# 0xC000005/PyChebyshev

Hardware: AMD Instinct MI355X
Metric: point-evals/sec, 5D Black-Scholes n=11^5 barycentric + TT, 1/2/4/8 GPU (higher is better)
Workload: dtype f64; 1 GPU; 5D Black-Scholes n=11^5 full-tensor barycentric, 1,000,000 fp64 queries per GPU; evals_per_point=1, parallelism=batch-sharded x1, model replicated, one process per GPU, gather=none

## Files before the change

### pychebyshev_amd/csrc/bary_kernels.h

```cpp
#pragma once

#include <type_traits>

#include "pcx_common.h"

static __global__ void k_mode_product(const double *__restrict__ in, double *__restrict__ out,
                               const double *__restrict__ D, long outer, int na, long inner) {
    long idx = (long)blockIdx.x * blockDim.x + threadIdx.x;
    long total = outer * na * inner;
    if (idx >= total) return;
    long q = idx % inner;
    long t = idx / inner;
    int i = (int)(t % na);
    long o = t / na;
    const double *src = in + (o * na) * inner + q;
    const double *drow = D + (long)i * na;
    double s = 0.0;
    for (int j = 0; j < na; ++j) s = __builtin_fma(src[(long)j * inner], drow[j], s);
    out[idx] = s;
}

static __global__ void k_contract_axis(const double *__restrict__ in, double *__restrict__ out,
                                const double *__restrict__ vec, long outer, int na, long inner) {
    long idx = (long)blockIdx.x * blockDim.x + threadIdx.x;
    if (idx >= outer * inner) return;
    long q = idx % inner;
    long o = idx / inner;
    const double *src = in + (o * na) * inner + q;
    double s = 0.0;
    for (int j = 0; j < na; ++j) s = __builtin_fma(src[(long)j * inner], vec[j], s);
    out[idx] = s;
}

static __global__ void k_pack_fragments(const double *__restrict__ T2, double *__restrict__ frag, int M,
                                 int K, int MT, int KS, int R) {
    long idx = (long)blockIdx.x * blockDim.x + threadIdx.x;
    long total = (long)MT * KS * 64;
    if (idx >= total) return;
    int l = (int)(idx & 63);
    long ts = idx >> 6;
    int s = (int)(ts % KS);
    int t = (int)(ts / KS);
    int m = 16 * t + (l & 15);
    int k = R + 4 * s + (l >> 4);
    frag[idx] = (m < M && k < K) ? T2[(long)m * K + k] : 0.0;
}

static __global__ void k_pack_seed(const double *__restrict__ T2, double *__restrict__ seed, int M, int K, int MT, int R, int tps) {
    long idx = (long)blockIdx.x * blockDim.x + threadIdx.x;
    if (idx >= (long)MT * 16 * R) return;
    const int j = (int)(idx & 3);
    const int r = (int)((idx >> 2) % R);
    const long tg = (idx >> 2) / R;
    const int g = (int)(tg & 3);
    const long t = tg >> 2;
    const long slab = tps > 0 ? t / tps : 0;
    const int m = 16 * (int)(tps > 0 ? t % tps : t) + g + 4 * j;
    seed[idx] = m < M ? T2[(slab * M + m) * K + r] : 0.0;
}

static __global__ void k_pack_fragments_slabs(const double *__restrict__ T3, double *__restrict__ frag, int n0, int M1,
                                       int K, int tps, int KS, int R) {
    long idx = (long)blockIdx.x * blockDim.x + threadIdx.x;
    const long per_slab = (long)tps * KS * 64;
    if (idx >= per_slab * n0) return;
    const int i0 = (int)(idx / per_slab);
    const long r = idx - (long)i0 * per_slab;
    int l = (int)(r & 63);
    long ts = r >> 6;
    int s = (int)(ts % KS);
    int t = (int)(ts / KS);
    int m = 16 * t + (l & 15);
    int k = R + 4 * s + (l >> 4);
    frag[idx] = (m < M1 && k < K) ? T3[((long)i0 * M1 + m) * K + k] : 0.0;
}

__device__ __forceinline__ void bary_g0_finish(const BaryG0 &gs, const double *__restrict__ diff0, double *vecA,
                                               double *vecB, const double *b0, int stride, double *out_row) {
    typedef const double __attribute__((address_space(4))) *cptr_t;
    const cptr_t D0 = (cptr_t)(unsigned long long)diff0;
    const int n0 = gs.n0;
    for (int o = 0; o <= gs.maxorder; ++o) {
        if (o > 0) {
            for (int i = 0; i < n0; ++i) {
                double s = 0.0;
                for (int j = 0; j < n0; ++j) s = __builtin_fma(vecA[j * stride], D0[i * n0 + j], s);
                vecB[i * stride] = s;
            }
            double *t = vecA; vecA = vecB; vecB = t;
        }
        double y = 0.0;
        for (int i = 0; i < n0; ++i) y = __builtin_fma(b0[i * stride], vecA[i * stride], y);
        if (out_row)
            for (int s = 0; s < gs.nmem; ++s)
                if (gs.order[s] == o) out_row[gs.col[s]] = y;
    }
}

__device__ __forceinline__ void bary_weights_1d(double x, const double *__restrict__ nodes,
                                                const double *__restrict__ wts, int n, double *dst,
                                                int stride) {
    int exact = -1;
    for (int j = 0; j < n; ++j) {
        double diff = x - nodes[j];
        if (exact < 0 && __builtin_fabs(diff) < 1e-14) exact = j;
    }
    if (exact >= 0) {
        for (int j = 0; j < n; ++j) dst[j * stride] = (j == exact) ? 1.0 : 0.0;
    } else {
        double su = 0.0;
        for (int j = 0; j < n; ++j) {
            double u = wts[j] / (x - nodes[j]);
            dst[j * stride] = u;
            su += u;
        }
        double r = 1.0 / su;
        for (int j = 0; j < n; ++j) dst[j * stride] *= r;
    }
}

__device__ __forceinline__ double code_weight(unsigned code, const double *bw_col, int PW) {
    double w0 = bw_col[(code & 255u) * PW];
    double w1 = bw_col[((code >> 8) & 255u) * PW];
    double w2 = bw_col[((code >> 16) & 255u) * PW];
    double w3 = bw_col[(code >> 24) * PW];
    return (w0 * w1) * (w2 * w3);
}

struct pcx_u4 { unsigned v[4]; };
__device__ __forceinline__ pcx_u4 load_row_codes(const unsigned *__restrict__ codes, long t, int g) {
    const uint4 q = reinterpret_cast<const uint4 *>(codes)[4 * t + g];
    return pcx_u4{{q.x, q.y, q.z, q.w}};
}

typedef const pcx_d4 __attribute__((address_space(1))) *pcx_seed_ptr;
template <int R>
struct pcx_seed { pcx_d4 v[R > 0 ? R : 1]; };
template <int R>
__device__ __forceinline__ pcx_seed<R> load_seed(pcx_seed_ptr seed, long t, int g) {
    pcx_seed<R> q;
#pragma unroll
    for (int r = 0; r < R; ++r) q.v[r] = seed[(4 * t + g) * R + r];
    return q;
}

__device__ __forceinline__ pcx_u4 load_row_offs(const unsigned *__restrict__ offs, long t, int g, int w) {
    const uint4 q = reinterpret_cast<const uint4 *>(offs)[8 * t + 2 * g + w];
    return pcx_u4{{q.x, q.y, q.z, q.w}};
}

template <int NF>
__device__ __forceinline__ double code_weight_t(unsigned code, const double *bw_col, int PW) {
    if constexpr (NF >= 4) return code_weight(code, bw_col, PW);
    else {
        double w0 = bw_col[(code & 255u) * PW];
        double w1 = bw_col[((code >> 8) & 255u) * PW];
        if constexpr (NF == 3) return (w0 * w1) * bw_col[((code >> 16) & 255u) * PW];
        else return w0 * w1;
    }
}

#define PCX_CHUNK_TILES 4

template <int KS, int NT, bool WIDE, int NF = 4, bool G0 = false, int R = 0>
__global__ void __launch_bounds__(256, 2)
k_bary_mfma(BaryDims dims, BaryMfmaPlan plan, const double *__restrict__ nodes,
            const double *__restrict__ wts, const double *const *__restrict__ frag_tab,
            const unsigned *__restrict__ rowcode, const unsigned *__restrict__ kcode,
            const unsigned *__restrict__ rowcode_hi, const unsigned *__restrict__ kcode_hi,
            const double *__restrict__ pts, double *__restrict__ out, long N, long ostride,
            long ooff, int chunks_per_split, double *__restrict__ partial,
            const int *__restrict__ perm, BaryG0 gs, const double *__restrict__ diff0,
            const unsigned *__restrict__ rowoff, BaryTail tail) {
    static_assert(NT == 1 || NT == 2 || NT == 4, "PW must divide the wave");
    constexpr int PW = 16 * NT;
    constexpr int PH = 64 / PW;
    extern __shared__ double lds[];
    const int lane = threadIdx.x & 63;
    const int wave = threadIdx.x >> 6;
    const int g = lane >> 4;
    const int c = lane & 15;
    double *bw = lds + (size_t)wave * plan.rows * PW;
    const double *bwt = bw + (size_t)plan.tail_base * PW;
    int bx = blockIdx.x;
    const int nchunks = (plan.MT + PCX_CHUNK_TILES - 1) / PCX_CHUNK_TILES;
    int ch0 = blockIdx.y * chunks_per_split, ch_len = chunks_per_split;
    bool split = gridDim.y > 1;
    long part_p0 = 0;
    long part_n = N;
    if (!G0 && tail.P > 0 && bx >= tail.first) {
        const int e = bx - tail.first;
        const int tb = e / tail.P;
        bx = tail.first + tb;
        ch0 = (e - tb * tail.P) * tail.cpp;
        ch_len = tail.cpp;
        split = true;
        part_p0 = (long)tail.first * 4 * PW;
        part_n = N - part_p0;
    }
    const int ch1 = (ch0 + ch_len < nchunks) ? ch0 + ch_len : nchunks;
    const long base = ((long)bx * 4 + wave) * PW;
    typedef const double __attribute__((address_space(1))) *gptr_t;
    const gptr_t frag = (gptr_t)frag_tab[blockIdx.z];
    const pcx_seed_ptr seed = (pcx_seed_ptr)(frag + (size_t)plan.MT * KS * 64);

    {
        const int pp = lane % PW;
        const int ph = lane / PW;
        const long pidx = base + pp;
        const bool valid = pidx < N;
        const long row = valid ? (perm ? (long)perm[pidx] : pidx) : 0;
        for (int k = ph; k < dims.d; k += PH) {
            const double *nd = nodes + dims.off[k];
            double x = valid ? pts[row * dims.d + k] : nd[0];
            const int trow = dims.off[k] + (k >= plan.split ? 1 : 0);
            bary_weights_1d(x, nd, wts + dims.off[k], dims.n[k], bw + (size_t)trow * PW + pp, PW);
        }
        if (ph == 0) {
            bw[(size_t)(plan.tail_base - 1) * PW + pp] = 1.0;
            bw[(size_t)(plan.rows - 1) * PW + pp] = 1.0;
        }
    }
    __syncthreads();

    double B[NT][KS];
    double ws[NT][R > 0 ? R : 1];
    auto tail_weights = [&](auto nft) {
        constexpr int NFT = decltype(nft)::value;
#pragma unroll
        for (int s = 0; s < KS; ++s) {
            unsigned code = kcode[4 * s + g];
#pragma unroll
            for (int nt = 0; nt < NT; ++nt) B[nt][s] = code_weight_t<NFT>(code, bwt + 16 * nt + c, PW);
            if (WIDE) {
                unsigned hi = kcode_hi[4 * s + g];
#pragma unroll
                for (int nt = 0; nt < NT; ++nt) B[nt][s] *= code_weight(hi, bwt + 16 * nt + c, PW);
            }
        }
#pragma unroll
        for (int r = 0; r < R; ++r) {
            unsigned code = kcode[4 * KS + r];
#pragma unroll
            for (int nt = 0; nt < NT; ++nt) ws[nt][r] = code_weight_t<NFT>(code, bwt + 16 * nt + c, PW);
            if (WIDE) {
                unsigned hi = kcode_hi[4 * KS + r];
#pragma unroll
                for (int nt = 0; nt < NT; ++nt) ws[nt][r] *= code_weight(hi, bwt + 16 * nt + c, PW);
            }
        }
    };
    if (!WIDE && dims.d - plan.split <= 2) tail_weights(std::integral_constant<int, 2>{});
    else tail_weights(std::integral_constant<int, 4>{});

    double total[NT], cs[NT];
#pragma unroll
    for (int nt = 0; nt < NT; ++nt) { total[nt] = 0.0; cs[nt] = 0.0; }
    const gptr_t tf = frag + lane;
    const int t_begin = ch0 * PCX_CHUNK_TILES;
    const int t_end = (ch1 * PCX_CHUNK_TILES < plan.MT) ? ch1 * PCX_CHUNK_TILES : plan.MT;
    constexpr bool PIPELINED = (KS >= 12);
    constexpr int DEPTH = 6;
    constexpr bool OFFS = PIPELINED && !WIDE && !G0;
    constexpr bool CODE2 = WIDE || (OFFS && NF >= 3);
    constexpr int CODE_STEP = 8;
    unsigned cc[4] = {0u, 0u, 0u, 0u}, cch[4] = {0u, 0u, 0u, 0u};
    auto load_codes = [&](long t) {
        const pcx_u4 q = OFFS ? load_row_offs(rowoff, t, g, 0) : load_row_codes(rowcode, t, g);
        pcx_u4 qh = q;
        if constexpr (WIDE) qh = load_row_codes(rowcode_hi, t, g);
        else if constexpr (CODE2) qh = load_row_offs(rowoff, t, g, 1);
#pragma unroll
        for (int j = 0; j < 4; ++j) {
            cc[j] = q.v[j];
            if (CODE2) cch[j] = qh.v[j];
        }
    };
    auto head_entry = [&](int j, int nt, int f) -> double {
        if constexpr (OFFS) {
            const unsigned word = f < 2 ? cc[j] : cch[j];
            const unsigned off = (f & 1) ? (word >> 16) : (word & 0xffffu);
            return *reinterpret_cast<const double *>(reinterpret_cast<const char *>(bw + 16 * nt + c) + off);
        } else {
            return bw[(size_t)((cc[j] >> (8 * f)) & 255u) * PW + 16 * nt + c];
        }
    };
    double head[DEPTH];
    pcx_d4 acc[NT];
    auto seed_acc = [&](const pcx_seed<R> &sd) {
#pragma unroll
        for (int nt = 0; nt < NT; ++nt) acc[nt] = (pcx_d4){0.0, 0.0, 0.0, 0.0};
#pragma unroll
        for (int r = 0; r < R; ++r)
#pragma unroll
            for (int nt = 0; nt < NT; ++nt)
#pragma unroll
                for (int j = 0; j < 4; ++j) acc[nt][j] = __builtin_fma(sd.v[r][j], ws[nt][r], acc[nt][j]);
    };
    constexpr bool CARRY = PIPELINED && R > 0;
#pragma unroll
    for (int i = 0; i < DEPTH; ++i) head[i] = 0.0;
    if (PIPELINED && t_begin < t_end) {
        if constexpr (R > 0) seed_acc(load_seed<R>(seed, t_begin, g));
        load_codes(t_begin);
#pragma unroll
        for (int i = 0; i < DEPTH; ++i) head[i] = tf[((size_t)t_begin * KS + i) * 64];
    }
    for (int t = t_begin; t < t_end; ++t) {
        double w[NT][4];
        pcx_seed<R> sdn;
        if constexpr (!CARRY) {
            if constexpr (R > 0) sdn = load_seed<R>(seed, t, g);
            seed_acc(sdn);
        }
        const gptr_t tt = tf + (size_t)t * KS * 64;
        if constexpr (PIPELINED) {
            const int t_next = (t + 1 < t_end) ? t + 1 : t;
            const gptr_t tn = tf + (size_t)t_next * KS * 64;
            double ring[DEPTH];
#pragma unroll
            for (int i = 0; i < DEPTH; ++i) ring[i] = head[i];
            double wr[4][NT][4];
            double wh[4][NT][4];
#pragma unroll
            for (int s = 0; s < KS; ++s) {
                const double a = ring[s % DEPTH];
                if (s + DEPTH < KS) ring[s % DEPTH] = tt[(s + DEPTH) * 64];
                else head[s + DEPTH - KS] = tn[(s + DEPTH - KS) * 64];
                if constexpr (R > 0) {
                    if (s == KS - DEPTH) sdn = load_seed<R>(seed, t_next, g);
                }
                if (s == CODE_STEP) load_codes(t_next);
#pragma unroll
                for (int j = 0; j < 4; ++j) {
                    if (s == 2 * j) {
#pragma unroll
                        for (int nt = 0; nt < NT; ++nt)
#pragma unroll
                            for (int f = 0; f < (NF < 4 ? NF : 4); ++f)
                                wr[j][nt][f] = head_entry(j, nt, f);
                    }
                    if (s == 2 * j + 2) {
#pragma unroll
                        for (int nt = 0; nt < NT; ++nt)
                            w[nt][j] = NF >= 4 ? (wr[j][nt][0] * wr[j][nt][1]) * (wr[j][nt][2] * wr[j][nt][3])
                                     : (NF == 3 ? (wr[j][nt][0] * wr[j][nt][1]) * wr[j][nt][2]
                                                : wr[j][nt][0] * wr[j][nt][1]);
                    }
                    if (WIDE && s == 2 * j + 1) {
#pragma unroll
                        for (int nt = 0; nt < NT; ++nt)
#pragma unroll
                            for (int f = 0; f < 4; ++f)
                                wh[j][nt][f] = bw[(size_t)((cch[j] >> (8 * f)) & 255u) * PW + 16 * nt + c];
                    }
                    if (WIDE && s == 2 * j + 3) {
#pragma unroll
                        for (int nt = 0; nt < NT; ++nt)
                            w[nt][j] *= (wh[j][nt][0] * wh[j][nt][1]) * (wh[j][nt][2] * wh[j][nt][3]);
                    }
                }
                __builtin_amdgcn_sched_barrier(0);
#pragma unroll
                for (int nt = 0; nt < NT; ++nt)
                    acc[nt] = __builtin_amdgcn_mfma_f64_16x16x4f64(a, B[nt][s], acc[nt], 0, 0, 0);
                __builtin_amdgcn_sched_barrier(0);
            }
        } else {
            const pcx_u4 q = load_row_codes(rowcode, t, g);
            pcx_u4 qh = q;
            if (WIDE) qh = load_row_codes(rowcode_hi, t, g);
#pragma unroll
            for (int j = 0; j < 4; ++j) {
                unsigned code = q.v[j];
#pragma unroll
                for (int nt = 0; nt < NT; ++nt) w[nt][j] = code_weight_t<NF>(code, bw + 16 * nt + c, PW);
                if (WIDE) {
                    unsigned hi = qh.v[j];
#pragma unroll
                    for (int nt = 0; nt < NT; ++nt) w[nt][j] *= code_weight(hi, bw + 16 * nt + c, PW);
                }
            }
#pragma unroll
            for (int s = 0; s < KS; ++s) {
                double a = tt[s * 64];
#pragma unroll
                for (int nt = 0; nt < NT; ++nt)
                    acc[nt] = __builtin_amdgcn_mfma_f64_16x16x4f64(a, B[nt][s], acc[nt], 0, 0, 0);
            }
        }
#pragma unroll
        for (int nt = 0; nt < NT; ++nt)
#pragma unroll
            for (int j = 0; j < 4; ++j) cs[nt] = __builtin_fma(acc[nt][j], w[nt][j], cs[nt]);
        if constexpr (CARRY) seed_acc(sdn);
        if constexpr (G0) {
            if ((t + 1) % gs.tps == 0) {
                const int i0 = t / gs.tps;
                double *Pl = const_cast<double *>(bwt);
#pragma unroll
                for (int nt = 0; nt < NT; ++nt) {
                    double v = cs[nt];
                    v += __shfl_xor(v, 16, 64);
                    v += __shfl_xor(v, 32, 64);
                    if (g == 0) Pl[(size_t)i0 * PW + 16 * nt + c] = v;
                    cs[nt] = 0.0;
                }
            }
            continue;
        }
        const bool chunk_end = ((t + 1) % PCX_CHUNK_TILES == 0) || (t + 1 == plan.MT);
        if (chunk_end) {
            if (split) {
                const int ch = t / PCX_CHUNK_TILES;
#pragma unroll
                for (int nt = 0; nt < NT; ++nt) {
                    long pidx = base + 16 * nt + c;
                    if (pidx < N)
                        partial[(((size_t)blockIdx.z * nchunks + ch) * 4 + g) * (size_t)part_n + (pidx - part_p0)] = cs[nt];
                }
            }
#pragma unroll
            for (int nt = 0; nt < NT; ++nt) { total[nt] += cs[nt]; cs[nt] = 0.0; }
        }
    }

    if constexpr (G0) {
        if (lane < PW) {
            double *Pl = const_cast<double *>(bwt) + lane;
            const long pidx = base + lane;
            const long row = (pidx < N) ? (perm ? (long)perm[pidx] : pidx) : 0;
            bary_g0_finish(gs, diff0, Pl, Pl + (size_t)gs.n0 * PW, bw + (size_t)dims.off[0] * PW + lane, PW,
                           pidx < N ? out + row * ostride + ooff : nullptr);
        }
        return;
    }
    if (!split) {
#pragma unroll
        for (int nt = 0; nt < NT; ++nt) {
            double v = total[nt];
            v += __shfl_xor(v, 16, 64);
            v += __shfl_xor(v, 32, 64);
            long pidx = base + 16 * nt + c;
            if (g == 0 && pidx < N) {
                long row = perm ? (long)perm[pidx] : pidx;
                out[row * ostride + ooff + blockIdx.z] = v;
            }
        }
    }
}

template <int KS, int R = 0>
__global__ void __launch_bounds__(512, 2)
k_bary_mfma4(BaryDims dims, BaryMfmaPlan plan, const double *__restrict__ nodes,
             const double *__restrict__ wts, const double *const *__restrict__ frag_tab,
             const unsigned *__restrict__ rowcode, const unsigned *__restrict__ kcode,
             const double *__restrict__ pts, double *__restrict__ out, long N, long ostride,
             long ooff, const int *__restrict__ perm) {
    constexpr int NT = 2;
    constexpr int PW = 32;
    constexpr int SLAB = KS * 64;
    constexpr int CPT = (SLAB + 511) / 512;
    extern __shared__ double lds[];
    const int lane = threadIdx.x & 63;
    const int wave = threadIdx.x >> 6;
    const int g = lane >> 4;
    const int c = lane & 15;
    double *bw = lds + (size_t)wave * plan.rows * PW;
    const double *bwt = bw + (size_t)plan.tail_base * PW;
    double *slab = lds + (size_t)8 * plan.rows * PW;
    const long base = ((long)blockIdx.x * 8 + wave) * PW;
    typedef const double __attribute__((address_space(1))) *gptr_t;
    const gptr_t frag = (gptr_t)frag_tab[blockIdx.z];
    const pcx_seed_ptr seed = (pcx_seed_ptr)(frag + (size_t)plan.MT * SLAB);

    {
        const int pp = lane & 31;
        const int ph = lane >> 5;
        const long pidx = base + pp;
        const bool valid = pidx < N;
        const long row = valid ? (perm ? (long)perm[pidx] : pidx) : 0;
        for (int k = ph; k < dims.d; k += 2) {
            const double *nd = nodes + dims.off[k];
            double x = valid ? pts[row * dims.d + k] : nd[0];
            const int trow = dims.off[k] + (k >= plan.split ? 1 : 0);
            bary_weights_1d(x, nd, wts + dims.off[k], dims.n[k], bw + (size_t)trow * PW + pp, PW);
        }
        if (ph == 0) {
            bw[(size_t)(plan.tail_base - 1) * PW + pp] = 1.0;
            bw[(size_t)(plan.rows - 1) * PW + pp] = 1.0;
        }
    }
    double stage[CPT];
    auto img_index = [](int i) {
        const int s_ = i >> 6, l_ = i & 63;
        const int k_ = l_ >> 4, rg_ = (l_ >> 2) & 3, ii_ = l_ & 3;
        return s_ * 64 + (rg_ >> 1) * 32 + (k_ * 4 + ii_) * 2 + (rg_ & 1);
    };
#pragma unroll
    for (int r = 0; r < CPT; ++r) {
        const int i = threadIdx.x + 512 * r;
        if (i < SLAB) slab[img_index(i)] = frag[i];
    }
    if (plan.MT > 1) {
#pragma unroll
        for (int r = 0; r < CPT; ++r) {
            const int i = threadIdx.x + 512 * r;
            stage[r] = (i < SLAB) ? frag[(size_t)SLAB + i] : 0.0;
        }
    }
    __syncthreads();

    double B[NT][KS];
#pragma unroll
    for (int s = 0; s < KS; ++s) {
        unsigned code = kcode[4 * s + g];
#pragma unroll
        for (int nt = 0; nt < NT; ++nt) B[nt][s] = code_weight(code, bwt + 16 * nt + c, PW);
    }
    double ws[NT][R > 0 ? R : 1];
#pragma unroll
    for (int r = 0; r < R; ++r) {
        unsigned code = kcode[4 * KS + r];
#pragma unroll
        for (int nt = 0; nt < NT; ++nt) ws[nt][r] = code_weight(code, bwt + 16 * nt + c, PW);
    }

    double total[NT], cs[NT];
#pragma unroll
    for (int nt = 0; nt < NT; ++nt) { total[nt] = 0.0; cs[nt] = 0.0; }
    const int aoff = ((lane >> 4) * 4 + (lane & 3)) * 2;
    for (int t = 0; t < plan.MT; ++t) {
        const double *cur = slab + (size_t)(t & 1) * SLAB;
        double *nxt = slab + (size_t)((t + 1) & 1) * SLAB;
        if (t + 1 < plan.MT) {
#pragma unroll
            for (int r = 0; r < CPT; ++r) {
                const int i = threadIdx.x + 512 * r;
                if (i < SLAB) nxt[img_index(i)] = stage[r];
            }
        }
        if (t + 2 < plan.MT) {
            const gptr_t src = frag + (size_t)(t + 2) * SLAB;
#pragma unroll
            for (int r = 0; r < CPT; ++r) {
                const int i = threadIdx.x + 512 * r;
                stage[r] = (i < SLAB) ? src[i] : 0.0;
            }
        }
        const pcx_u4 q4 = load_row_codes(rowcode, t, g);
        const unsigned code0 = q4.v[0], code1 = q4.v[1], code2 = q4.v[2], code3 = q4.v[3];
        pcx_seed<R> sd;
        if constexpr (R > 0) sd = load_seed<R>(seed, t, g);
#pragma unroll
        for (int half = 0; half < 2; ++half) {
            constexpr int DEPTH = (KS < 6) ? KS : 6;
            double acc[2][NT];
#pragma unroll
            for (int r = 0; r < 2; ++r)
#pragma unroll
                for (int nt = 0; nt < NT; ++nt) {
                    acc[r][nt] = 0.0;
#pragma unroll
                    for (int rr = 0; rr < R; ++rr) acc[r][nt] = __builtin_fma(sd.v[rr][2 * half + r], ws[nt][rr], acc[r][nt]);
                }
            typedef double d2_t __attribute__((ext_vector_type(2)));
            const d2_t *ar = reinterpret_cast<const d2_t *>(cur + aoff + 32 * half);
            d2_t ring[DEPTH];
#pragma unroll
            for (int s = 0; s < DEPTH; ++s) ring[s] = ar[s * 32];
#pragma unroll
            for (int s = 0; s < KS; ++s) {
                const double a0 = ring[s % DEPTH][0], a1 = ring[s % DEPTH][1];
                if (s + DEPTH < KS) ring[s % DEPTH] = ar[(s + DEPTH) * 32];
                __builtin_amdgcn_sched_barrier(0);
#pragma unroll
                for (int nt = 0; nt < NT; ++nt) {
                    acc[0][nt] = __builtin_amdgcn_mfma_f64_4x4x4f64(a0, B[nt][s], acc[0][nt], 0, 0, 0);
                    acc[1][nt] = __builtin_amdgcn_mfma_f64_4x4x4f64(a1, B[nt][s], acc[1][nt], 0, 0, 0);
                }
                __builtin_amdgcn_sched_barrier(0);
            }
            const unsigned codeA = half ? code2 : code0, codeB = half ? code3 : code1;
#pragma unroll
            for (int nt = 0; nt < NT; ++nt) {
                cs[nt] = __builtin_fma(acc[0][nt], code_weight(codeA, bw + 16 * nt + c, PW), cs[nt]);
                cs[nt] = __builtin_fma(acc[1][nt], code_weight(codeB, bw + 16 * nt + c, PW), cs[nt]);
            }
        }
        const bool chunk_end = ((t + 1) % PCX_CHUNK_TILES == 0) || (t + 1 == plan.MT);
        if (chunk_end) {
#pragma unroll
            for (int nt = 0; nt < NT; ++nt) { total[nt] += cs[nt]; cs[nt] = 0.0; }
        }
        __syncthreads();
    }

#pragma unroll
    for (int nt = 0; nt < NT; ++nt) {
        double v = total[nt];
        v += __shfl_xor(v, 16, 64);
        v += __shfl_xor(v, 32, 64);
        long pidx = base + 16 * nt + c;
        if (g == 0 && pidx < N) {
            long row = perm ? (long)perm[pidx] : pidx;
            out[row * ostride + ooff + blockIdx.z] = v;
        }
    }
}

static __global__ void __launch_bounds__(256)
k_bary_reduce(const double *__restrict__ partial, double *__restrict__ out, long N, int nchunks, int nspec,
              long ostride, long ooff, const int *__restrict__ perm, long p0) {
    __shared__ double sg[4][64];
    const int lane = threadIdx.x & 63;
    const int g = threadIdx.x >> 6;
    const long idx = (long)blockIdx.x * 64 + lane;
    const bool valid = idx < N * nspec;
    const long p = valid ? idx % N : 0;
    const int z = valid ? (int)(idx / N) : 0;
    const double *src = partial + ((size_t)z * nchunks * 4 + g) * (size_t)N + p;
    const size_t step = (size_t)4 * (size_t)N;
    double t = 0.0;
    int ch = 0;
    for (; ch + 8 <= nchunks; ch += 8) {
        double v[8];
#pragma unroll
        for (int i = 0; i < 8; ++i) v[i] = src[(size_t)(ch + i) * step];
#pragma unroll
        for (int i = 0; i < 8; ++i) t += v[i];
    }
    for (; ch < nchunks; ++ch) t += src[(size_t)ch * step];
    sg[g][lane] = t;
    __syncthreads();
    if (g == 0 && valid) {
        long row = perm ? (long)perm[p0 + p] : p0 + p;
        out[row * ostride + ooff + z] = (sg[0][lane] + sg[1][lane]) + (sg[2][lane] + sg[3][lane]);
    }
}

static __global__ void __launch_bounds__(256)
k_bary_rows(BaryDims dims, int LPP, const double *__restrict__ nodes,
            const double *__restrict__ wts, const double *__restrict__ T,
            const double *__restrict__ pts, double *__restrict__ out, long N, long ostride,
            long ooff, const int *__restrict__ perm) {
    extern __shared__ double lds[];
    const int ppw = 256 / LPP;
    const int pl = threadIdx.x / LPP;
    const int sub = threadIdx.x % LPP;
    const long pidx = (long)blockIdx.x * ppw + pl;
    const bool valid = pidx < N;
    const long row = valid ? (perm ? (long)perm[pidx] : pidx) : 0;
    double *bw = lds + (size_t)pl * dims.sum_n;
    for (int k = sub; k < dims.d; k += LPP) {
        const double *nd = nodes + dims.off[k];
        double x = valid ? pts[row * dims.d + k] : nd[0];
        bary_weights_1d(x, nd, wts + dims.off[k], dims.n[k], bw + dims.off[k], 1);
    }
    __syncthreads();
    const int d = dims.d;
    const int K = dims.n[d - 1];
    long M = 1;
    for (int k = 0; k < d - 1; ++k) M *= dims.n[k];
    const double *bl = bw + dims.off[d - 1];
    double acc = 0.0;
    for (long m = sub; m < M; m += LPP) {
        double w = 1.0;
        long rem = m;
        for (int k = d - 2; k >= 0; --k) {
            int nk = dims.n[k];
            int i = (int)(rem % nk);
            rem /= nk;
            w *= bw[dims.off[k] + i];
        }
        const double *row = T + m * K;
        double s = 0.0;
        for (int j = 0; j < K; ++j) s = __builtin_fma(row[j], bl[j], s);
        acc = __builtin_fma(s, w, acc);
    }
    for (int o = LPP >> 1; o > 0; o >>= 1) acc += __shfl_xor(acc, o, 64);
    if (sub == 0 && valid) out[row * ostride + ooff] = acc;
}


typedef const double __attribute__((address_space(4))) *pcx_cptr;
__device__ __forceinline__ pcx_cptr pcx_as_constant(const double *p) { return (pcx_cptr)(unsigned long long)p; }

template <int NLP, bool EXACT>
__device__ __forceinline__ void bary_weights_reg(double x, double scale, pcx_cptr snodes, pcx_cptr wts, int n,
                                                 double (&b)[NLP]) {
    double t[NLP];
    double run = 1.0, amin = 1.0e300;
#pragma unroll
    for (int j = 0; j < NLP; ++j) {
        b[j] = 0.0;
        t[j] = 1.0;
        if (EXACT || j < n) {
            t[j] = __builtin_fma(x, scale, -snodes[j]);
            amin = __builtin_fmin(amin, __builtin_fabs(t[j]));
            b[j] = wts[j] * run;
            run *= t[j];
        }
    }
    run = 1.0;
    double su = 0.0;
#pragma unroll
    for (int j = NLP - 1; j >= 0; --j) {
        if (EXACT || j < n) {
            b[j] *= run;
            su += b[j];
            run *= t[j];
        }
    }
    const double r = 1.0 / su;
#pragma unroll
    for (int j = 0; j < NLP; ++j) b[j] *= r;
    if (amin < 1e-14 * scale) {
        bool found = false;
#pragma unroll
        for (int j = 0; j < NLP; ++j) {
            const bool hit = !found && (EXACT || j < n) && __builtin_fabs(t[j]) < 1e-14 * scale;
            b[j] = hit ? 1.0 : 0.0;
            found = found || hit;
        }
    }
}

__device__ __forceinline__ void bary_weights_prod(double x, double scale, pcx_cptr snodes, pcx_cptr wts, int n,
                                                  double *dst, int stride) {
    double run = 1.0, amin = 1.0e300;
    for (int j = 0; j < n; ++j) {
        dst[j * stride] = wts[j] * run;
        const double t = __builtin_fma(x, scale, -snodes[j]);
        amin = __builtin_fmin(amin, __builtin_fabs(t));
        run *= t;
    }
    run = 1.0;
    double su = 0.0;
    for (int j = n - 1; j >= 0; --j) {
        const double c = dst[j * stride] * run;
        dst[j * stride] = c;
        su += c;
        run *= __builtin_fma(x, scale, -snodes[j]);
    }
    const double r = 1.0 / su;
    for (int j = 0; j < n; ++j) dst[j * stride] *= r;
    if (amin < 1e-14 * scale) {
        bool found = false;
        for (int j = 0; j < n; ++j) {
            const bool hit = !found && __builtin_fabs(__builtin_fma(x, scale, -snodes[j])) < 1e-14 * scale;
            dst[j * stride] = hit ? 1.0 : 0.0;
            found = found || hit;
        }
    }
}

template <int LEVEL, int DOUT, int NLP>
__device__ __forceinline__ double bary_small_nest(const BaryDims &dims, pcx_cptr Tb,
                                                  const double *bw_lane, const double (&bl)[NLP]) {
    if constexpr (LEVEL == DOUT) {
        double s = 0.0;
#pragma unroll
        for (int i = 0; i < NLP; ++i) s = __builtin_fma(Tb[i], bl[i], s);
        return s;
    } else {
        long stride = 1;
        for (int q = LEVEL + 1; q <= DOUT; ++q) stride *= dims.n[q];
        const double *wk = bw_lane + (size_t)dims.off[LEVEL] * 64;
        double s = 0.0;
        for (int i = 0; i < dims.n[LEVEL]; ++i)
            s = __builtin_fma(wk[(size_t)i * 64], bary_small_nest<LEVEL + 1, DOUT, NLP>(dims, Tb + i * stride, bw_lane, bl), s);
        return s;
    }
}


template <int DOUT, int NLP>
__device__ __forceinline__ void bary_small_body(const BaryDims &dims, const BarySmallScale &sc, pcx_cptr csn, pcx_cptr cnd,
                                                pcx_cptr cw, const double *T, const double *const *T_tab, int m,
                                                const double *__restrict__ pts, double *__restrict__ out, bool valid,
                                                long row, long ostride, long ooff, double *bw_lane) {
    const int d = DOUT + 1;
#pragma unroll
    for (int k = 0; k < DOUT; ++k) {
        const double x = valid ? pts[row * d + k] : cnd[dims.off[k]];
        bary_weights_prod(x, sc.s[k], csn + dims.off[k], cw + dims.off[k], dims.n[k],
                          bw_lane + (size_t)dims.off[k] * 64, 64);
    }
    double bl[NLP];
    {
        const double x = valid ? pts[row * d + DOUT] : cnd[dims.off[DOUT]];
        if (dims.n[DOUT] == NLP)
            bary_weights_reg<NLP, true>(x, sc.s[DOUT], csn + dims.off[DOUT], cw + dims.off[DOUT], NLP, bl);
        else
            bary_weights_reg<NLP, false>(x, sc.s[DOUT], csn + dims.off[DOUT], cw + dims.off[DOUT], dims.n[DOUT], bl);
    }
    if (T_tab == nullptr) {
        const double y = bary_small_nest<0, DOUT, NLP>(dims, pcx_as_constant(T), bw_lane, bl);
        if (valid) out[row * ostride + ooff] = y;
    } else {
        for (int z = 0; z < m; ++z) {
            const double y = bary_small_nest<0, DOUT, NLP>(dims, pcx_as_constant(T_tab[z]), bw_lane, bl);
            if (valid) out[row * ostride + ooff + z] = y;
        }
    }
}

template <int DOUT, int NLP>
__global__ void __launch_bounds__(64)
k_bary_small(BaryDims dims, BarySmallScale sc, const double *__restrict__ snodes, const double *__restrict__ nodes,
             const double *__restrict__ wts, const double *__restrict__ T, const double *const *__restrict__ T_tab,
             int m, const double *__restrict__ pts, double *__restrict__ out, long N, long ostride, long ooff,
             const int *__restrict__ perm) {
    extern __shared__ double lds[];
    const int lane = threadIdx.x;
    const long pidx = (long)blockIdx.x * 64 + lane;
    const bool valid = pidx < N;
    const long row = valid ? (perm ? (long)perm[pidx] : pidx) : 0;
    bary_small_body<DOUT, NLP>(dims, sc, pcx_as_constant(snodes), pcx_as_constant(nodes), pcx_as_constant(wts), T, T_tab, m,
                               pts, out, valid, row, ostride, ooff, lds + lane);
}

template <int NL>
__device__ __forceinline__ double bary_sq_block(pcx_cptr Tb, const double (&b1)[NL], const double (&b2)[NL]) {
    constexpr int R4 = (NL % 4 == 0) ? 4 : (NL % 3 == 0) ? 3 : (NL % 5 == 0) ? 5 : (NL % 4 == 1 && NL > 5) ? 3 : 4;
    double t0 = 0.0, t1 = 0.0;
#pragma unroll
    for (int i = 0; i < NL; i += R4) {
        double s[R4];
#pragma unroll
        for (int r = 0; r < R4; ++r)
            if (i + r < NL) s[r] = Tb[(i + r) * NL] * b2[0];
#pragma unroll
        for (int k = 1; k < NL; ++k)
#pragma unroll
            for (int r = 0; r < R4; ++r)
                if (i + r < NL) s[r] = __builtin_fma(Tb[(i + r) * NL + k], b2[k], s[r]);
#pragma unroll
        for (int r = 0; r < R4; ++r)
            if (i + r < NL) {
                if (r & 1) t1 = __builtin_fma(b1[i + r], s[r], t1);
                else t0 = __builtin_fma(b1[i + r], s[r], t0);
            }
    }
    return t0 + t1;
}

template <int NL, int LEAD>
__device__ __forceinline__ double bary_sq_tensor(const BaryDims &dims, pcx_cptr T, const double *bw_lane,
                                                 const double (&b1)[NL], const double (&b2)[NL]) {
    if constexpr (LEAD == 0) return bary_sq_block<NL>(T, b1, b2);
    else if constexpr (LEAD == 1) {
        double y = 0.0;
        for (int i0 = 0; i0 < dims.n[0]; ++i0, T += NL * NL)
            y = __builtin_fma(bw_lane[(size_t)i0 * 64], bary_sq_block<NL>(T, b1, b2), y);
        return y;
    } else {
        double y = 0.0;
        const double *w1 = bw_lane + (size_t)dims.off[1] * 64;
        for (int i0 = 0; i0 < dims.n[0]; ++i0) {
            double a = 0.0;
            for (int i1 = 0; i1 < dims.n[1]; ++i1, T += NL * NL)
                a = __builtin_fma(w1[(size_t)i1 * 64], bary_sq_block<NL>(T, b1, b2), a);
            y = __builtin_fma(bw_lane[(size_t)i0 * 64], a, y);
        }
        return y;
    }
}

template <int NL, int LEAD>
__device__ __forceinline__ void bary_sq_body(const BaryDims &dims, const BarySmallScale &sc, pcx_cptr csn, pcx_cptr cnd, pcx_cptr cw,
                                             const double *T, const double *const *T_tab, int m, const double *__restrict__ pts,
                                             double *__restrict__ out, bool valid, long row, long ostride, long ooff,
                                             double *bw_lane) {
    constexpr int D = LEAD + 2;
#pragma unroll
    for (int k = 0; k < LEAD; ++k) {
        const double x = valid ? pts[row * D + k] : cnd[dims.off[k]];
        bary_weights_prod(x, sc.s[k], csn + dims.off[k], cw + dims.off[k], dims.n[k], bw_lane + (size_t)dims.off[k] * 64, 64);
    }
    double b1[NL], b2[NL];
    {
        const double x1 = valid ? pts[row * D + LEAD] : cnd[dims.off[LEAD]];
        const double x2 = valid ? pts[row * D + LEAD + 1] : cnd[dims.off[LEAD + 1]];
        bary_weights_reg<NL, true>(x1, sc.s[LEAD], csn + dims.off[LEAD], cw + dims.off[LEAD], NL, b1);
        bary_weights_reg<NL, true>(x2, sc.s[LEAD + 1], csn + dims.off[LEAD + 1], cw + dims.off[LEAD + 1], NL, b2);
    }
    for (int z = 0; z < m; ++z) {
        const double y = bary_sq_tensor<NL, LEAD>(dims, pcx_as_constant(T_tab ? T_tab[z] : T), bw_lane, b1, b2);
        if (valid) out[row * ostride + ooff + z] = y;
    }
}

template <int NL, int LEAD>
__global__ void __launch_bounds__(64)
k_bary_sq(BaryDims dims, BarySmallScale sc, const double *__restrict__ snodes, const double *__restrict__ nodes,
          const double *__restrict__ wts, const double *__restrict__ T, const double *const *__restrict__ T_tab, int m,
          const double *__restrict__ pts, double *__restrict__ out, long N, long ostride, long ooff,
          const int *__restrict__ perm) {
    extern __shared__ double lds[];
    const int lane = threadIdx.x;
    const long pidx = (long)blockIdx.x * 64 + lane;
    const bool valid = pidx < N;
    const long row = valid ? (perm ? (long)perm[pidx] : pidx) : 0;
    bary_sq_body<NL, LEAD>(dims, sc, pcx_as_constant(snodes), pcx_as_constant(nodes), pcx_as_constant(wts), T, T_tab, m, pts, out,
                           valid, row, ostride, ooff, lds + lane);
}


template <int DOUT, int NLP>
__global__ void __launch_bounds__(64)
k_bary_small_pieces(BaryDims dims, const SplinePieceModel *__restrict__ models, const int *__restrict__ blk_piece,
                    const int *__restrict__ blk_first, const int *__restrict__ piece_end, int m,
                    const double *__restrict__ pts, double *__restrict__ out, long ostride, long ooff,
                    const int *__restrict__ perm) {
    extern __shared__ double lds[];
    const int lane = threadIdx.x;
    const int piece = blk_piece[blockIdx.x];
    const long pidx = (long)blk_first[blockIdx.x] + lane;
    const bool valid = pidx < (long)piece_end[piece];
    const long row = valid ? (long)perm[pidx] : 0;
    typedef const SplinePieceModel __attribute__((address_space(4))) *model_cptr;
    const model_cptr mp = (model_cptr)(unsigned long long)(models + piece);
    BarySmallScale sc;
#pragma unroll
    for (int k = 0; k < 4; ++k) sc.s[k] = mp->sc.s[k];
    bary_small_body<DOUT, NLP>(dims, sc, pcx_as_constant(mp->snodes), pcx_as_constant(mp->nodes), pcx_as_constant(mp->wts),
                               mp->T, mp->T_tab, m, pts, out, valid, row, ostride, ooff, lds + lane);
}

template <int NL, int LEAD>
__global__ void __launch_bounds__(64)
k_bary_sq_pieces(BaryDims dims, const SplinePieceModel *__restrict__ models, const int *__restrict__ blk_piece,
                 const int *__restrict__ blk_first, const int *__restrict__ piece_end, int m,
                 const double *__restrict__ pts, double *__restrict__ out, long ostride, long ooff,
                 const int *__restrict__ perm) {
    extern __shared__ double lds[];
    const int lane = threadIdx.x;
    const int piece = blk_piece[blockIdx.x];
    const long pidx = (long)blk_first[blockIdx.x] + lane;
    const bool valid = pidx < (long)piece_end[piece];
    const long row = valid ? (long)perm[pidx] : 0;
    typedef const SplinePieceModel __attribute__((address_space(4))) *model_cptr;
    const model_cptr mp = (model_cptr)(unsigned long long)(models + piece);
    BarySmallScale sc;
#pragma unroll
    for (int k = 0; k < 4; ++k) sc.s[k] = mp->sc.s[k];
    bary_sq_body<NL, LEAD>(dims, sc, pcx_as_constant(mp->snodes), pcx_as_constant(mp->nodes), pcx_as_constant(mp->wts), mp->T,
                           mp->T_tab, m, pts, out, valid, row, ostride, ooff, lds + lane);
}
```

Baseline: 211.3 million point-evals/s.

## Use buffer loads with scalar bases and double-buffer MFMA accumulators across tiles

The pipelined MFMA barycentric kernel now loads fragments, seeds and row codes through AMD buffer resources built from wave-uniform (readfirstlane) bases. Offsets become immediate or scalar values, which is meant to cut per-lane 64-bit address arithmetic. A new deferred path for the offset-code case alternates two accumulator sets, so one tile's weighted reduction and seed initialization overlap with the next tile's MFMAs instead of stalling on them. This raises register pressure and adds code complexity, and the seed base assumes seeds sit directly after the fragments in memory.

```diff
diff --git a/pychebyshev_amd/csrc/bary_kernels.h b/pychebyshev_amd/csrc/bary_kernels.h
--- a/pychebyshev_amd/csrc/bary_kernels.h
+++ b/pychebyshev_amd/csrc/bary_kernels.h
@@ -144,9 +144,38 @@
     return q;
 }
 
-__device__ __forceinline__ pcx_u4 load_row_offs(const unsigned *__restrict__ offs, long t, int g, int w) {
-    const uint4 q = reinterpret_cast<const uint4 *>(offs)[8 * t + 2 * g + w];
-    return pcx_u4{{q.x, q.y, q.z, q.w}};
+
+typedef __amdgpu_buffer_rsrc_t pcx_rsrc;
+__device__ __forceinline__ const char *pcx_uniform(const void *p) {
+    const unsigned long long a = (unsigned long long)p;
+    const unsigned lo = __builtin_amdgcn_readfirstlane((unsigned)a);
+    const unsigned hi = __builtin_amdgcn_readfirstlane((unsigned)(a >> 32));
+    return (const char *)(((unsigned long long)hi << 32) | lo);
+}
+template <unsigned TILE>
+__device__ __forceinline__ pcx_rsrc buffer_window(const char *p, int tiles, int t) {
+    const unsigned left = (unsigned)(tiles - t);
+    const unsigned held = left < 0xffffffffu / TILE ? left : 0xffffffffu / TILE;
+    return __builtin_amdgcn_make_buffer_rsrc(const_cast<char *>(p + (size_t)t * TILE), 0, (int)(held * TILE), 0x00020000);
+}
+__device__ __forceinline__ double buffer_f64(pcx_rsrc rs, int voff, int soff) {
+    return __builtin_bit_cast(double, __builtin_amdgcn_raw_buffer_load_b64(rs, voff, soff, 0));
+}
+__device__ __forceinline__ pcx_u4 buffer_u4(pcx_rsrc rs, int voff, int soff) {
+    const auto q = __builtin_amdgcn_raw_buffer_load_b128(rs, voff, soff, 0);
+    return pcx_u4{{q[0], q[1], q[2], q[3]}};
+}
+template <int R>
+__device__ __forceinline__ pcx_seed<R> buffer_seed(pcx_rsrc rs, int voff) {
+    pcx_seed<R> q;
+#pragma unroll
+    for (int r = 0; r < R; ++r) {
+        const auto lo = __builtin_amdgcn_raw_buffer_load_b128(rs, voff, 32 * r, 0);
+        const auto hi = __builtin_amdgcn_raw_buffer_load_b128(rs, voff, 32 * r + 16, 0);
+        typedef unsigned u8v __attribute__((ext_vector_type(8)));
+        q.v[r] = __builtin_bit_cast(pcx_d4, (u8v){lo[0], lo[1], lo[2], lo[3], hi[0], hi[1], hi[2], hi[3]});
+    }
+    return q;
 }
 
 template <int NF>
@@ -264,12 +293,21 @@
     constexpr bool OFFS = PIPELINED && !WIDE && !G0;
     constexpr bool CODE2 = WIDE || (OFFS && NF >= 3);
     constexpr int CODE_STEP = 8;
+    constexpr unsigned FRAG_TILE = KS * 512, SEED_TILE = 128 * (R > 0 ? R : 1), CODE_TILE = OFFS ? 128 : 64;
+    const char *const ufrag = PIPELINED ? pcx_uniform((const double *)frag) : nullptr;
+    const char *const useed = PIPELINED ? ufrag + (size_t)plan.MT * FRAG_TILE : nullptr;
+    const char *const ucode = PIPELINED ? pcx_uniform(OFFS ? rowoff : rowcode) : nullptr;
+    const char *const ucode_hi = (PIPELINED && WIDE) ? pcx_uniform(rowcode_hi) : nullptr;
+    const int frag_lane = lane * 8, seed_lane = g * 32 * R, code_lane = g * (int)(CODE_TILE / 4);
+    auto frag_window = [&](int t) { return buffer_window<FRAG_TILE>(ufrag, plan.MT, t); };
+    auto seed_window = [&](int t) { return buffer_window<SEED_TILE>(useed, plan.MT, t); };
     unsigned cc[4] = {0u, 0u, 0u, 0u}, cch[4] = {0u, 0u, 0u, 0u};
-    auto load_codes = [&](long t) {
-        const pcx_u4 q = OFFS ? load_row_offs(rowoff, t, g, 0) : load_row_codes(rowcode, t, g);
+    auto load_codes = [&](int t) {
+        const pcx_rsrc cw = buffer_window<CODE_TILE>(ucode, plan.MT, t);
+        const pcx_u4 q = buffer_u4(cw, code_lane, 0);
         pcx_u4 qh = q;
-        if constexpr (WIDE) qh = load_row_codes(rowcode_hi, t, g);
-        else if constexpr (CODE2) qh = load_row_offs(rowoff, t, g, 1);
+        if constexpr (WIDE) qh = buffer_u4(buffer_window<CODE_TILE>(ucode_hi, plan.MT, t), code_lane, 0);
+        else if constexpr (CODE2) qh = buffer_u4(cw, code_lane, 16);
 #pragma unroll
         for (int j = 0; j < 4; ++j) {
             cc[j] = q.v[j];
@@ -301,11 +339,107 @@
 #pragma unroll
     for (int i = 0; i < DEPTH; ++i) head[i] = 0.0;
     if (PIPELINED && t_begin < t_end) {
-        if constexpr (R > 0) seed_acc(load_seed<R>(seed, t_begin, g));
+        if constexpr (R > 0) seed_acc(buffer_seed<R>(seed_window(t_begin), seed_lane));
         load_codes(t_begin);
-#pragma unroll
-        for (int i = 0; i < DEPTH; ++i) head[i] = tf[((size_t)t_begin * KS + i) * 64];
-    }
+        const pcx_rsrc fw = frag_window(t_begin);
+#pragma unroll
+        for (int i = 0; i < DEPTH; ++i) head[i] = buffer_f64(fw, frag_lane, i * 512);
+    }
+    constexpr bool DEFER = OFFS && NT * KS <= 64;
+    if constexpr (DEFER) {
+        pcx_d4 acc2[NT];
+        double w[NT][4];
+#pragma unroll
+        for (int nt = 0; nt < NT; ++nt) {
+            if constexpr (R == 0) acc[nt] = (pcx_d4){0.0, 0.0, 0.0, 0.0};
+            acc2[nt] = (pcx_d4){0.0, 0.0, 0.0, 0.0};
+#pragma unroll
+            for (int j = 0; j < 4; ++j) w[nt][j] = 0.0;
+        }
+        auto add_tile = [&](pcx_d4 (&a)[NT]) {
+#pragma unroll
+            for (int nt = 0; nt < NT; ++nt)
+#pragma unroll
+                for (int j = 0; j < 4; ++j) cs[nt] = __builtin_fma(a[nt][j], w[nt][j], cs[nt]);
+        };
+        auto end_chunk = [&](int t) {
+            if (split) {
+                const int ch = t / PCX_CHUNK_TILES;
+#pragma unroll
+                for (int nt = 0; nt < NT; ++nt) {
+                    long pidx = base + 16 * nt + c;
+                    if (pidx < N)
+                        partial[(((size_t)blockIdx.z * nchunks + ch) * 4 + g) * (size_t)part_n + (pidx - part_p0)] = cs[nt];
+                }
+            }
+#pragma unroll
+            for (int nt = 0; nt < NT; ++nt) { total[nt] += cs[nt]; cs[nt] = 0.0; }
+        };
+        auto tile = [&](int t, pcx_d4 (&cur)[NT], pcx_d4 (&idle)[NT]) {
+            const int t_next = (t + 1 < t_end) ? t + 1 : t;
+            const pcx_rsrc ft = frag_window(t), fn = frag_window(t_next);
+            pcx_seed<R> sdn;
+            double ring[DEPTH];
+#pragma unroll
+            for (int i = 0; i < DEPTH; ++i) ring[i] = head[i];
+            double wr[4][NT][4];
+#pragma unroll
+            for (int s = 0; s < KS; ++s) {
+                const double a = ring[s % DEPTH];
+                if (s + DEPTH < KS) ring[s % DEPTH] = buffer_f64(ft, frag_lane, (s + DEPTH) * 512);
+                else head[s + DEPTH - KS] = buffer_f64(fn, frag_lane, (s + DEPTH - KS) * 512);
+                if constexpr (R > 0) {
+                    if (s == KS - DEPTH) sdn = buffer_seed<R>(seed_window(t_next), seed_lane);
+                }
+                if (s == CODE_STEP) load_codes(t_next);
+                if (s == 1) {
+                    add_tile(idle);
+                    if (t > t_begin && t % PCX_CHUNK_TILES == 0) end_chunk(t - 1);
+                }
+#pragma unroll
+                for (int j = 0; j < 4; ++j) {
+                    if (s == 2 * j) {
+#pragma unroll
+                        for (int nt = 0; nt < NT; ++nt)
+#pragma unroll
+                            for (int f = 0; f < (NF < 4 ? NF : 4); ++f) wr[j][nt][f] = head_entry(j, nt, f);
+                    }
+                    if (s == 2 * j + 2) {
+#pragma unroll
+                        for (int nt = 0; nt < NT; ++nt)
+                            w[nt][j] = NF >= 4 ? (wr[j][nt][0] * wr[j][nt][1]) * (wr[j][nt][2] * wr[j][nt][3])
+                                     : (NF == 3 ? (wr[j][nt][0] * wr[j][nt][1]) * wr[j][nt][2]
+                                                : wr[j][nt][0] * wr[j][nt][1]);
+                    }
+                }
+                __builtin_amdgcn_sched_barrier(0);
+#pragma unroll
+                for (int nt = 0; nt < NT; ++nt)
+                    cur[nt] = __builtin_amdgcn_mfma_f64_16x16x4f64(a, B[nt][s], cur[nt], 0, 0, 0);
+                __builtin_amdgcn_sched_barrier(0);
+            }
+#pragma unroll
+            for (int nt = 0; nt < NT; ++nt) idle[nt] = (pcx_d4){0.0, 0.0, 0.0, 0.0};
+#pragma unroll
+            for (int r = 0; r < R; ++r)
+#pragma unroll
+                for (int nt = 0; nt < NT; ++nt)
+#pragma unroll
+                    for (int j = 0; j < 4; ++j) idle[nt][j] = __builtin_fma(sdn.v[r][j], ws[nt][r], idle[nt][j]);
+        };
+        int t = t_begin;
+        for (; t + 1 < t_end; t += 2) {
+            tile(t, acc, acc2);
+            tile(t + 1, acc2, acc);
+        }
+        if (t < t_end) {
+            tile(t, acc, acc2);
+            add_tile(acc);
+        } else if (t_begin < t_end) {
+            add_tile(acc2);
+        }
+        if (t_begin < t_end) end_chunk(t_end - 1);
+    } else
     for (int t = t_begin; t < t_end; ++t) {
         double w[NT][4];
         pcx_seed<R> sdn;
@@ -313,10 +447,9 @@
             if constexpr (R > 0) sdn = load_seed<R>(seed, t, g);
             seed_acc(sdn);
         }
-        const gptr_t tt = tf + (size_t)t * KS * 64;
         if constexpr (PIPELINED) {
             const int t_next = (t + 1 < t_end) ? t + 1 : t;
-            const gptr_t tn = tf + (size_t)t_next * KS * 64;
+            const pcx_rsrc ft = frag_window(t), fn = frag_window(t_next);
             double ring[DEPTH];
 #pragma unroll
             for (int i = 0; i < DEPTH; ++i) ring[i] = head[i];
@@ -325,10 +458,10 @@
 #pragma unroll
             for (int s = 0; s < KS; ++s) {
                 const double a = ring[s % DEPTH];
-                if (s + DEPTH < KS) ring[s % DEPTH] = tt[(s + DEPTH) * 64];
-                else head[s + DEPTH - KS] = tn[(s + DEPTH - KS) * 64];
+                if (s + DEPTH < KS) ring[s % DEPTH] = buffer_f64(ft, frag_lane, (s + DEPTH) * 512);
+                else head[s + DEPTH - KS] = buffer_f64(fn, frag_lane, (s + DEPTH - KS) * 512);
                 if constexpr (R > 0) {
-                    if (s == KS - DEPTH) sdn = load_seed<R>(seed, t_next, g);
+                    if (s == KS - DEPTH) sdn = buffer_seed<R>(seed_window(t_next), seed_lane);
                 }
                 if (s == CODE_STEP) load_codes(t_next);
 #pragma unroll
@@ -367,6 +500,7 @@
                 __builtin_amdgcn_sched_barrier(0);
             }
         } else {
+            const gptr_t tt = tf + (size_t)t * KS * 64;
             const pcx_u4 q = load_row_codes(rowcode, t, g);
             pcx_u4 qh = q;
             if (WIDE) qh = load_row_codes(rowcode_hi, t, g);
```

New measurement: 214.3 million point-evals/s, median of 6. +1.4%, better.
